# cthadeufaria/computer-vision-shoplifting-detection

Measured on AMD Instinct MI355X. Metric: frames/s @640x640, higher is better.
Workload: dtype f32; 1 GPU; yolov8n 640x640 synthetic BGR frames (512 distinct frames per GPU), batch 512/GPU/step, predict conf=0.25 iou=0.7 max_det=300 (letterbox+stem, conv graph, decode, NMS, rows to host); global_batch=512, params=3151904, parallelism=frame-sharded dp1, ranks=1, collective_world_size=1, activation_bytes_per_gpu=10027008000

## Files before the change

### computer-vision-shoplifting-detection_amd/csrc/conv_f32_sparse.hip

```cpp
#include "conv_f32.h"
#include <algorithm>

#pragma clang fp contract(off)

namespace mi355 {

__device__ __forceinline__ void sp_append(bool flag, int* list, int cap, int* count, int* overflow, int v) {
    const unsigned long long m = __ballot(flag);
    if (m == 0ull) return;
    const int lane = threadIdx.x & 63, leader = __ffsll((long long)m) - 1;
    int base = 0;
    if (lane == leader) base = atomicAdd(count, __popcll(m));
    base = __shfl(base, leader);
    const int pos = base + __popcll(m & ((1ull << lane) - 1ull));
    if (flag) {
        if (pos < cap) list[pos] = v;
        else *overflow = 1;
    }
}

__global__ __launch_bounds__(256) void sparse_lists_kernel(SparseArgs a) {
    const int b = blockIdx.y, an = blockIdx.x * 256 + threadIdx.x;
    const bool live = an < a.A;
    int l = 0;
#pragma unroll
    for (int j = 1; j < 3; ++j)
        if (j < a.n_levels && an >= a.lv[j].anchor0) l = j;
    const int H = a.lv[l].H, W = a.lv[l].W, a0 = a.lv[l].anchor0;
    bool cand = false, dil = false;
    const int li = live ? an - a0 : 0;
    if (live) {
        const int y = li / W, x = li - y * W;
        const float2* best = a.best + (size_t)b * a.A + a0;
        for (int dy = -1; dy <= 1; ++dy)
            for (int dx = -1; dx <= 1; ++dx) {
                const int yy = y + dy, xx = x + dx;
                if ((unsigned)yy >= (unsigned)H || (unsigned)xx >= (unsigned)W) continue;
                const float2 bc = best[yy * W + xx];
                bool ok = bc.x > a.conf;
                if (ok && a.class_mask) { const int c = (int)bc.y; ok = (a.class_mask[c >> 5] >> (c & 31)) & 1u; }
                dil |= ok;
                if (dy == 0 && dx == 0) cand = ok;
            }
    }
    const int v = b * H * W + li;
    for (int j = 0; j < a.n_levels; ++j) {
        sp_append(dil && l == j, a.lv[j].dil, a.lv[j].cap_dil, a.state + j, a.state + 8, v);
        sp_append(cand && l == j, a.lv[j].cand, a.lv[j].cap_cand, a.state + 4 + j, a.state + 8, v);
    }
}

__device__ __forceinline__ void sp_conv3x3_64(const float* map, int cs, int cib, int H, int W, int b, int y, int x, const float* wpk,
                                              int lane, f32x4 (&tot)[4]) {
    const int g = lane >> 4;
    const float* base = map + (size_t)b * H * W * cs + 4 * g;
    int off[9]; bool inb[9];
#pragma unroll
    for (int k = 0; k < 9; ++k) {
        const int yy = y + k / 3 - 1, xx = x + k % 3 - 1;
        inb[k] = (unsigned)yy < (unsigned)H && (unsigned)xx < (unsigned)W;
        off[k] = inb[k] ? (yy * W + xx) * cs : 0;
    }
#pragma unroll
    for (int ct = 0; ct < 4; ++ct) tot[ct] = (f32x4){0.f, 0.f, 0.f, 0.f};
    const float* wl = wpk + lane * 4;
    const size_t wct = (size_t)9 * cib * 256;
    for (int cb = 0; cb < cib; ++cb) {
        f32x4 xv[9];
#pragma unroll
        for (int k = 0; k < 9; ++k) {
            xv[k] = *(const f32x4*)(base + off[k] + 16 * cb);
            if (!inb[k]) xv[k] = (f32x4){0.f, 0.f, 0.f, 0.f};
        }
        f32x4 acc[4];
#pragma unroll
        for (int k = 0; k < 9; ++k) {
            f32x4 w[4];
#pragma unroll
            for (int ct = 0; ct < 4; ++ct) w[ct] = *(const f32x4*)(wl + ct * wct + ((size_t)k * cib + cb) * 256);
#pragma unroll
            for (int s = 0; s < 4; ++s)
#pragma unroll
                for (int ct = 0; ct < 4; ++ct)
                    acc[ct] = __builtin_amdgcn_mfma_f32_16x16x4f32(w[ct][s], xv[k][s], (k == 0 && s == 0) ? (f32x4){0.f, 0.f, 0.f, 0.f} : acc[ct], 0, 0, 0);
        }
#pragma unroll
        for (int ct = 0; ct < 4; ++ct) tot[ct] += acc[ct];
    }
}

__device__ __forceinline__ int sp_entry(const int* list, int n, int t0, int lane, bool* ok) {
    const int e = t0 + (lane & 15);
    *ok = e < n;
    return list[e < n ? e : n - 1];
}

__global__ __launch_bounds__(256) void sparse_conv_a_kernel(SparseArgs a) {
    if (a.state[8]) return;
    const int l = blockIdx.y;
    const SparseLevel& L = a.lv[l];
    const int n = min(a.state[l], L.cap_dil);
    if ((int)blockIdx.x * 64 >= n) return;
    const int lane = threadIdx.x & 63, wave = __builtin_amdgcn_readfirstlane(threadIdx.x >> 6);
    const int t0 = (blockIdx.x * 4 + wave) * 16;
    if (t0 >= n) return;
    bool ok;
    const int v = sp_entry(L.dil, n, t0, lane, &ok);
    const int HW = L.H * L.W, b = v / HW, li = v - b * HW, y = li / L.W, x = li - y * L.W;
    f32x4 tot[4];
    sp_conv3x3_64(L.src, L.src_cs, L.cib, L.H, L.W, b, y, x, L.wA, lane, tot);
    if (!ok) return;
    float* dst = L.mid + (size_t)v * L.mid_cs + (lane >> 4) * 4;
#pragma unroll
    for (int ct = 0; ct < 4; ++ct) {
        f32x4 r = tot[ct] + *(const f32x4*)(L.biasA + ct * 16 + (lane >> 4) * 4);
        r = act4(r, a.act);
        *(f32x4*)(dst + ct * 16) = r;
    }
}

constexpr int SP_LDP = 68;

__global__ __launch_bounds__(256) void sparse_conv_b_kernel(SparseArgs a) {
    __shared__ __attribute__((aligned(16))) float logits[4][16 * SP_LDP];
    if (a.state[8]) return;
    const int l = blockIdx.y;
    const SparseLevel& L = a.lv[l];
    const int n = min(a.state[4 + l], L.cap_cand);
    const int lane = threadIdx.x & 63, wave = __builtin_amdgcn_readfirstlane(threadIdx.x >> 6);
    const int g = lane >> 4, p = lane & 15;
    const int t0 = (blockIdx.x * 4 + wave) * 16;
    if (t0 >= n) return;
    bool ok;
    const int v = sp_entry(L.cand, n, t0, lane, &ok);
    const int HW = L.H * L.W, b = v / HW, li = v - b * HW, y = li / L.W, x = li - y * L.W;
    f32x4 tot[4];
    sp_conv3x3_64(L.mid, L.mid_cs, 4, L.H, L.W, b, y, x, L.wB, lane, tot);
    f32x4 x2[4];
#pragma unroll
    for (int ct = 0; ct < 4; ++ct) x2[ct] = act4(tot[ct] + *(const f32x4*)(L.biasB + ct * 16 + g * 4), a.act);
    float* lg = logits[wave];
#pragma unroll
    for (int ct2 = 0; ct2 < 4; ++ct2) {
        f32x4 tot2 = (f32x4){0.f, 0.f, 0.f, 0.f};
#pragma unroll
        for (int cb = 0; cb < 4; ++cb) {
            const f32x4 w = *(const f32x4*)(L.wC + ((size_t)ct2 * 4 + cb) * 256 + lane * 4);
            f32x4 p2;
#pragma unroll
            for (int s = 0; s < 4; ++s)
                p2 = __builtin_amdgcn_mfma_f32_16x16x4f32(w[s], x2[cb][s], s == 0 ? (f32x4){0.f, 0.f, 0.f, 0.f} : p2, 0, 0, 0);
            tot2 += p2;
        }
        const f32x4 r = tot2 + *(const f32x4*)(L.biasC + ct2 * 16 + g * 4);
        *(f32x4*)(lg + p * SP_LDP + ct2 * 16 + g * 4) = r;
    }
    __builtin_amdgcn_fence(__ATOMIC_RELEASE, "workgroup");
    __builtin_amdgcn_wave_barrier();
    __builtin_amdgcn_fence(__ATOMIC_ACQUIRE, "workgroup");
    float side[16];
#pragma unroll
    for (int j = 0; j < 4; ++j) {
        const f32x4 q = *(const f32x4*)(lg + p * SP_LDP + 16 * g + 4 * j);
        side[4 * j] = q[0]; side[4 * j + 1] = q[1]; side[4 * j + 2] = q[2]; side[4 * j + 3] = q[3];
    }
    const float d = det_dfl_side(side);
    const float d0 = __shfl(d, p), d1 = __shfl(d, p + 16), d2 = __shfl(d, p + 32), d3 = __shfl(d, p + 48);
    if (ok && g == 0) {
        const float4 o = det_dist2bbox(d0, d1, d2, d3, (float)x + 0.5f, (float)y + 0.5f, (float)L.stride);
        float* out = a.pred + ((size_t)b * a.A + L.anchor0 + li) * a.no;
        if ((a.no & 3) == 0) *(float4*)out = o;
        else { out[0] = o.x; out[1] = o.y; out[2] = o.z; out[3] = o.w; }
    }
}

const char* launch_sparse_lists(const SparseArgs& a, hipStream_t st) {
    hipLaunchKernelGGL(sparse_lists_kernel, dim3((unsigned)((a.A + 255) / 256), (unsigned)a.B), dim3(256), 0, st, a);
    hipError_t e = hipGetLastError();
    return e == hipSuccess ? nullptr : hipGetErrorString(e);
}

const char* launch_sparse_box(const SparseArgs& a, hipStream_t st) {
    int cap_d = 0, cap_c = 0;
    for (int l = 0; l < a.n_levels; ++l) { cap_d = std::max(cap_d, a.lv[l].cap_dil); cap_c = std::max(cap_c, a.lv[l].cap_cand); }
    hipLaunchKernelGGL(sparse_conv_a_kernel, dim3((unsigned)((cap_d + 63) / 64), (unsigned)a.n_levels), dim3(256), 0, st, a);
    hipLaunchKernelGGL(sparse_conv_b_kernel, dim3((unsigned)((cap_c + 63) / 64), (unsigned)a.n_levels), dim3(256), 0, st, a);
    hipError_t e = hipGetLastError();
    return e == hipSuccess ? nullptr : hipGetErrorString(e);
}

}
```

Baseline: 13140 frames/s.

## Build sparse candidate lists per frame with LDS bitmap and block-level prefix scan

```diff
diff --git a/computer-vision-shoplifting-detection_amd/csrc/conv_f32_sparse.hip b/computer-vision-shoplifting-detection_amd/csrc/conv_f32_sparse.hip
--- a/computer-vision-shoplifting-detection_amd/csrc/conv_f32_sparse.hip
+++ b/computer-vision-shoplifting-detection_amd/csrc/conv_f32_sparse.hip
@@ -5,48 +5,99 @@
 
 namespace mi355 {
 
-__device__ __forceinline__ void sp_append(bool flag, int* list, int cap, int* count, int* overflow, int v) {
-    const unsigned long long m = __ballot(flag);
-    if (m == 0ull) return;
-    const int lane = threadIdx.x & 63, leader = __ffsll((long long)m) - 1;
-    int base = 0;
-    if (lane == leader) base = atomicAdd(count, __popcll(m));
-    base = __shfl(base, leader);
-    const int pos = base + __popcll(m & ((1ull << lane) - 1ull));
-    if (flag) {
-        if (pos < cap) list[pos] = v;
-        else *overflow = 1;
-    }
-}
-
-__global__ __launch_bounds__(256) void sparse_lists_kernel(SparseArgs a) {
-    const int b = blockIdx.y, an = blockIdx.x * 256 + threadIdx.x;
-    const bool live = an < a.A;
+constexpr int SP_LIST_THREADS = 1024, SP_LIST_WAVES = SP_LIST_THREADS / 64;
+constexpr int SP_MAX_ANCHORS = 65536 / 8 * 64;
+
+__device__ __forceinline__ bool sp_bit(const unsigned long long* bm, int i) { return (bm[i >> 6] >> (i & 63)) & 1ull; }
+
+__device__ __forceinline__ void sp_flags(const SparseArgs& a, const unsigned long long* bm, int b, int an, int* l_, int* v_, bool* cand_,
+                                         bool* dil_) {
     int l = 0;
 #pragma unroll
     for (int j = 1; j < 3; ++j)
         if (j < a.n_levels && an >= a.lv[j].anchor0) l = j;
-    const int H = a.lv[l].H, W = a.lv[l].W, a0 = a.lv[l].anchor0;
     bool cand = false, dil = false;
-    const int li = live ? an - a0 : 0;
-    if (live) {
-        const int y = li / W, x = li - y * W;
-        const float2* best = a.best + (size_t)b * a.A + a0;
+    int v = 0;
+    if (an < a.A) {
+        const int H = a.lv[l].H, W = a.lv[l].W, a0 = a.lv[l].anchor0;
+        const int li = an - a0, y = li / W, x = li - y * W;
+        cand = sp_bit(bm, an);
         for (int dy = -1; dy <= 1; ++dy)
             for (int dx = -1; dx <= 1; ++dx) {
                 const int yy = y + dy, xx = x + dx;
                 if ((unsigned)yy >= (unsigned)H || (unsigned)xx >= (unsigned)W) continue;
-                const float2 bc = best[yy * W + xx];
-                bool ok = bc.x > a.conf;
-                if (ok && a.class_mask) { const int c = (int)bc.y; ok = (a.class_mask[c >> 5] >> (c & 31)) & 1u; }
-                dil |= ok;
-                if (dy == 0 && dx == 0) cand = ok;
+                dil |= sp_bit(bm, a0 + yy * W + xx);
             }
-    }
-    const int v = b * H * W + li;
-    for (int j = 0; j < a.n_levels; ++j) {
-        sp_append(dil && l == j, a.lv[j].dil, a.lv[j].cap_dil, a.state + j, a.state + 8, v);
-        sp_append(cand && l == j, a.lv[j].cand, a.lv[j].cap_cand, a.state + 4 + j, a.state + 8, v);
+        v = b * H * W + li;
+    }
+    *l_ = l; *v_ = v; *cand_ = cand; *dil_ = dil;
+}
+
+__global__ __launch_bounds__(SP_LIST_THREADS) void sparse_lists_kernel(SparseArgs a) {
+    extern __shared__ unsigned long long sp_bm[];
+    __shared__ int wcnt[SP_LIST_WAVES][6], wbase[SP_LIST_WAVES][6];
+    const int b = blockIdx.x, lane = threadIdx.x & 63, wave = threadIdx.x >> 6;
+    const int a64 = (a.A + 63) & ~63;
+    const int per = (((a.A + SP_LIST_WAVES - 1) / SP_LIST_WAVES) + 63) & ~63;
+    const int r0 = wave * per, r1 = min(r0 + per, a64);
+    const float2* best = a.best + (size_t)b * a.A;
+    for (int c0 = r0; c0 < r1; c0 += 64) {
+        const int an = c0 + lane;
+        bool ok = false;
+        if (an < a.A) {
+            const float2 bc = best[an];
+            ok = bc.x > a.conf;
+            if (ok && a.class_mask) { const int c = (int)bc.y; ok = (a.class_mask[c >> 5] >> (c & 31)) & 1u; }
+        }
+        const unsigned long long m = __ballot(ok);
+        if (lane == 0) sp_bm[c0 >> 6] = m;
+    }
+    __syncthreads();
+    int cnt[6] = {0, 0, 0, 0, 0, 0};
+    for (int c0 = r0; c0 < r1; c0 += 64) {
+        int l, v; bool cand, dil;
+        sp_flags(a, sp_bm, b, c0 + lane, &l, &v, &cand, &dil);
+#pragma unroll
+        for (int j = 0; j < 3; ++j) {
+            cnt[j] += __popcll(__ballot(dil && l == j));
+            cnt[3 + j] += __popcll(__ballot(cand && l == j));
+        }
+    }
+    if (lane == 0)
+#pragma unroll
+        for (int k = 0; k < 6; ++k) wcnt[wave][k] = cnt[k];
+    __syncthreads();
+    if (threadIdx.x < 6) {
+        const int k = threadIdx.x;
+        int tot = 0;
+        for (int w = 0; w < SP_LIST_WAVES; ++w) { wbase[w][k] = tot; tot += wcnt[w][k]; }
+        const int seg = tot ? atomicAdd(a.state + (k / 3) * 4 + k % 3, tot) : 0;
+        for (int w = 0; w < SP_LIST_WAVES; ++w) wbase[w][k] += seg;
+    }
+    __syncthreads();
+    int run[6];
+#pragma unroll
+    for (int k = 0; k < 6; ++k) run[k] = wbase[wave][k];
+    const unsigned long long below = (1ull << lane) - 1ull;
+    for (int c0 = r0; c0 < r1; c0 += 64) {
+        int l, v; bool cand, dil;
+        sp_flags(a, sp_bm, b, c0 + lane, &l, &v, &cand, &dil);
+#pragma unroll
+        for (int j = 0; j < 3; ++j) {
+            if (j >= a.n_levels) break;
+            const unsigned long long md = __ballot(dil && l == j), mc = __ballot(cand && l == j);
+            if (dil && l == j) {
+                const int pos = run[j] + __popcll(md & below);
+                if (pos < a.lv[j].cap_dil) a.lv[j].dil[pos] = v;
+                else a.state[8] = 1;
+            }
+            if (cand && l == j) {
+                const int pos = run[3 + j] + __popcll(mc & below);
+                if (pos < a.lv[j].cap_cand) a.lv[j].cand[pos] = v;
+                else a.state[8] = 1;
+            }
+            run[j] += __popcll(md); run[3 + j] += __popcll(mc);
+        }
     }
 }
 
@@ -175,7 +226,9 @@
 }
 
 const char* launch_sparse_lists(const SparseArgs& a, hipStream_t st) {
-    hipLaunchKernelGGL(sparse_lists_kernel, dim3((unsigned)((a.A + 255) / 256), (unsigned)a.B), dim3(256), 0, st, a);
+    if (a.A > SP_MAX_ANCHORS) return "sparse box branch: more anchors per frame than the lists kernel's bitmap holds";
+    const size_t lds = (size_t)((a.A + 63) / 64) * 8;
+    hipLaunchKernelGGL(sparse_lists_kernel, dim3((unsigned)a.B), dim3(SP_LIST_THREADS), lds, st, a);
     hipError_t e = hipGetLastError();
     return e == hipSuccess ? nullptr : hipGetErrorString(e);
 }
```

Result: no change. 13170 frames/s (median of 5 runs) (+0.3%).
